# Krual-T/OutfitX

Hardware: AMD Instinct MI355X
Metric: outfits/sec CP forward (8-item sets, 224^2, bf16) (higher is better)
Workload: dtype f16

## Files before the change

outfitx_amd/csrc/fused_qkv_attn.hip:

```cpp
#include "attn_wave.h"
#include "gemm_common.h"

namespace {

struct FusedK {
    const char* X;
    const char* Wqkv;
    char* out;
    const float* bias;
    const float* row_stat;
    const float* col_sum;
    int n_img, S, Wm, heads, ldx, ldo, G, nwg;
    float scale;
    const char* W8 = nullptr; const char* scale8 = nullptr;
};

constexpr int FQ_TM = 256, FQ_TN = 192, FQ_STAGE = (FQ_TM + FQ_TN) * BK * 2;
constexpr int FQ_QK_ROW = 144;
constexpr int FQ_NT = 4;
static_assert(FQ_TN == 3 * ATTN_D && 16 * FQ_NT == ATTN_D, "the tail runs the attention core at NT = 4 on one head's 64 q, 64 k and 64 v columns");
constexpr int FQ_Q_OFF = 0, FQ_K_OFF = FQ_TM * FQ_QK_ROW, FQ_V_OFF = 2 * FQ_TM * FQ_QK_ROW;
constexpr int FQ_LDS = 2 * FQ_STAGE + 16 * ATTN_V_ROW;
constexpr int FQ2_BK = 32, FQ2_A = FQ_TM * FQ2_BK * 2, FQ2_W = FQ_TN * FQ2_BK * 2, FQ2_STAGE = FQ2_A + 2 * FQ2_W, FQ2_NST = 3;
constexpr int FQ2_LDS = FQ2_NST * FQ2_STAGE;
static_assert(FQ2_LDS >= FQ_LDS, "q | k | v image must fit the dual-weight stages");
constexpr int FQ8_A = FQ_TM * 32 * 2, FQ8_W = FQ_TN * 32 * 2, FQ8_STAGE = FQ8_A + FQ8_W, FQ8_NST = 4;
constexpr int FQ8_W8BASE = FQ8_NST * FQ8_STAGE, FQ8_W8 = FQ_TN * 128;
constexpr int FQ8_IMG = FQ8_STAGE, FQ8_CST = FQ8_IMG + FQ_LDS, FQ8_CST_WAVE = (2 * 64 + 2 * 96) * 4;
constexpr int FQ8_LDS = FQ8_CST + 8 * FQ8_CST_WAVE;
static_assert(FQ8_CST >= FQ8_W8BASE + FQ8_W8 && FQ8_IMG + 2 * FQ_STAGE >= FQ8_W8BASE + FQ8_W8, "the V pad rows and the constants lie behind everything LDS-DMA fills");
static_assert(FQ8_LDS <= 160 * 1024, "one block per CU");

template <typename T>
__device__ __forceinline__ void fq_attention(OFX_LDS char* lds, const FusedK& p, int wave, int lane, int m0, int head);

template <typename T, bool W2 = false>
__global__ __launch_bounds__(512, 2) void fused_qkv_attn_kernel(FusedK p) {
    typedef typename OpT<T>::v8 v8;
    typedef typename OpT<T>::v4 v4;
    extern __shared__ __attribute__((aligned(16))) char smem[];
    OFX_LDS char* lds = (OFX_LDS char*)smem;
    const int tid = threadIdx.x, lane = tid & 63;
    const int wave = __builtin_amdgcn_readfirstlane(tid >> 6);
    const int wr = wave >> 2, wc = wave & 3;

    const int bid = xcd_remap(blockIdx.x, p.nwg);
    const int hh = p.heads % 2 == 0 ? p.heads / 2 : p.heads, halves = p.heads / hh, per_unit = 6 * hh;
    const int unit = bid / per_unit, in_unit = bid % per_unit;
    const int grp = (unit / halves) * 6 + in_unit / hh, head = (unit % halves) * hh + in_unit % hh;
    if (grp * p.G >= p.n_img) return;
    const int M = p.n_img * p.S;
    const int m0 = grp * p.G * p.S;
    const int n_live_img = min(p.G, p.n_img - grp * p.G);

    f32x4 acc[8][3];
#pragma unroll
    for (int i = 0; i < 8; ++i)
#pragma unroll
        for (int j = 0; j < 3; ++j) acc[i][j] = f32x4{0.f, 0.f, 0.f, 0.f};
    const int fr = lane & 15, fq = lane >> 4;

    if constexpr (W2) {
    const PpLane32 L(lane);
    const int prow = L.prow, pchk = L.pchk;
    const char* a_base = p.X + (size_t)m0 * p.ldx * 2;
    const char* w_base = p.Wqkv + (size_t)head * 64 * (2 * p.Wm) * 2;
    unsigned a_off[2], w_off[3];
#pragma unroll
    for (int i = 0; i < 2; ++i) {
        const int row = (wave * 2 + i) * 16 + prow;
        const int rr = m0 + row < M ? row : M - 1 - m0;
        a_off[i] = ((unsigned)rr * p.ldx + pchk * 8) * 2;
    }
    int w_dst[3];
#pragma unroll
    for (int i = 0; i < 3; ++i) {
        const int q = wave * 3 + i;
        const int row = (q % 12) * 16 + prow;
        const unsigned grow = (unsigned)(row >> 6) * p.Wm + (row & 63);
        w_off[i] = (grow * (2 * p.Wm) + (q >= 12 ? p.Wm : 0) + pchk * 8) * 2;
        w_dst[i] = FQ2_A + (q >= 12 ? FQ2_W : 0) + (q % 12) * 1024;
    }
    const int a_dst = wave * 2 * 1024;
    const int nk = p.Wm / FQ2_BK;
    auto issue_all = [&](int step) {
        const int sc = step < nk ? step : nk - 1;
        OFX_LDS char* base = lds + (step % FQ2_NST) * FQ2_STAGE;
        const char* ak = a_base + (size_t)sc * FQ2_BK * 2;
        const char* wk = w_base + (size_t)sc * FQ2_BK * 2;
#pragma unroll
        for (int i = 0; i < 2; ++i) glds16(ak + a_off[i], base + a_dst + i * 1024);
#pragma unroll
        for (int i = 0; i < 3; ++i) glds16(wk + w_off[i], base + w_dst[i]);
    };
    const int a_frag = (wr * 128 + fr) * 64 + L.fchk;
    const int w_frag = FQ2_A + (wc * 48 + fr) * 64 + L.fchk;
    v8 af[8], wh[3], wl[3];
    auto read = [&](int t) { pp_w2_read<3>(lds + (t % FQ2_NST) * FQ2_STAGE, a_frag, w_frag, FQ2_W, af, wh, wl); };
    auto mfma = [&] { pp_w2_mfma<T, 3>(acc, af, wh, wl); };
    issue_all(0); issue_all(1);
    asm volatile("s_waitcnt vmcnt(5)" ::: "memory");
    __builtin_amdgcn_s_barrier();
    if (wr == 0) {
        for (int t = 0; t < nk; ++t) pp_slot<0, 5>([&] { issue_all(t + 2); }, [&] { read(t); }, mfma);
        pp_group_end<0>();
    } else {
        pp_group_begin<1>();
        for (int t = 0; t < nk; ++t) pp_slot<1, 5>([&] { issue_all(t + 2); }, [&] { read(t); }, mfma);
    }
    asm volatile("s_waitcnt vmcnt(0)" ::: "memory");
    __builtin_amdgcn_s_barrier();
    if (tid < 16 * ATTN_V_ROW / 16) *(OFX_LDS f32x4*)(lds + 2 * FQ_STAGE + tid * 16) = f32x4{0.f, 0.f, 0.f, 0.f};
    } else {
    if (tid < 16 * ATTN_V_ROW / 16) *(OFX_LDS f32x4*)(lds + 2 * FQ_STAGE + tid * 16) = f32x4{0.f, 0.f, 0.f, 0.f};

    const int lrow = lane >> 3, lchk = lane & 7;
    const char* a_base = p.X + (size_t)m0 * p.ldx * 2;
    const char* w_base = p.Wqkv + (size_t)head * 64 * p.Wm * 2;
    unsigned a_off[4], w_off[3];
#pragma unroll
    for (int i = 0; i < 4; ++i) {
        const int row = (wave * 4 + i) * 8 + lrow;
        const int rr = m0 + row < M ? row : M - 1 - m0;
        a_off[i] = ((unsigned)rr * p.ldx + (lchk ^ ((row >> 1) & 7)) * 8) * 2;
    }
#pragma unroll
    for (int i = 0; i < 3; ++i) {
        const int row = (wave * 3 + i) * 8 + lrow;
        const unsigned grow = (unsigned)(row >> 6) * p.Wm + (row & 63);
        w_off[i] = (grow * p.Wm + (lchk ^ ((row >> 1) & 7)) * 8) * 2;
    }
    const int a_dst = wave * 4 * 1024, w_dst = FQ_TM * BK * 2 + wave * 3 * 1024;
    auto issue_all = [&](int kt, int stage) {
        OFX_LDS char* base = lds + stage * FQ_STAGE;
        const char* ak = a_base + (size_t)kt * BK * 2;
        const char* wk = w_base + (size_t)kt * BK * 2;
#pragma unroll
        for (int i = 0; i < 4; ++i) glds16(ak + a_off[i], base + a_dst + i * 1024);
#pragma unroll
        for (int i = 0; i < 3; ++i) glds16(wk + w_off[i], base + w_dst + i * 1024);
    };

    const int fsw = fr >> 1;
    const int a_frag = (wr * 128 + fr) * 128;
    const int w_frag = FQ_TM * BK * 2 + (wc * 48 + fr) * 128;
    v8 af[2][8], wf[2][3];

#define FQ_READ_FRAGS(STG)                                                                                    \
    {                                                                                                         \
        OFX_LDS char* base_ = lds + (STG) * FQ_STAGE;                                                         \
        _Pragma("unroll") for (int ks = 0; ks < 2; ++ks) {                                                    \
            const int chk = ((ks * 4 + fq) ^ fsw) * 16;                                                       \
            _Pragma("unroll") for (int j = 0; j < 3; ++j) wf[ks][j] = *(OFX_LDS v8*)(base_ + w_frag + j * 16 * 128 + chk); \
            _Pragma("unroll") for (int i = 0; i < 8; ++i) af[ks][i] = *(OFX_LDS v8*)(base_ + a_frag + i * 16 * 128 + chk); \
        }                                                                                                     \
    }

    const int nk = p.Wm / BK;
    issue_all(0, 0);
    issue_all(nk > 1 ? 1 : 0, 1);
    asm volatile("s_waitcnt vmcnt(7)" ::: "memory");
    __builtin_amdgcn_s_barrier();
    if (wr == 0) {
        for (int t = 0; t < nk; ++t) {
            if (t >= 1 && t + 1 < nk) issue_all(t + 1, (t + 1) & 1);
            FQ_READ_FRAGS(t & 1)
            asm volatile("s_waitcnt lgkmcnt(0)" ::: "memory");
            __builtin_amdgcn_s_barrier();
            __builtin_amdgcn_s_setprio(1);
#pragma unroll
            for (int m = 0; m < 48; ++m) {
                const int ks = m / 24, i = (m % 24) / 3, j = m % 3;
                acc[i][j] = OpT<T>::mfma16(wf[ks][j], af[ks][i], acc[i][j]);
            }
            __builtin_amdgcn_s_setprio(0);
            asm volatile("s_waitcnt vmcnt(0)" ::: "memory");
            __builtin_amdgcn_s_barrier();
        }
        __builtin_amdgcn_s_barrier();
    } else {
        __builtin_amdgcn_s_barrier();
        for (int t = 0; t < nk; ++t) {
            FQ_READ_FRAGS(t & 1)
            asm volatile("s_waitcnt vmcnt(0)" ::: "memory");
            asm volatile("s_waitcnt lgkmcnt(0)" ::: "memory");
            __builtin_amdgcn_s_barrier();
            OFX_LDS char* nbase = lds + (t & 1) * FQ_STAGE;
            const int kn = t + 2 < nk ? t + 2 : nk - 1;
            const char* ak = a_base + (size_t)kn * BK * 2;
            const char* wk = w_base + (size_t)kn * BK * 2;
            __builtin_amdgcn_s_setprio(1);
#pragma unroll
            for (int m = 0; m < 48; ++m) {
                if (m % 6 == 0 && m / 6 < 7) {
                    const int q = m / 6;
                    if (q < 4) glds16(ak + a_off[q], nbase + a_dst + q * 1024);
                    else glds16(wk + w_off[q - 4], nbase + w_dst + (q - 4) * 1024);
                }
                const int ks = m / 24, i = (m % 24) / 3, j = m % 3;
                acc[i][j] = OpT<T>::mfma16(wf[ks][j], af[ks][i], acc[i][j]);
            }
            __builtin_amdgcn_s_setprio(0);
            __builtin_amdgcn_s_barrier();
        }
    }
#undef FQ_READ_FRAGS
    asm volatile("s_waitcnt vmcnt(0)" ::: "memory");
    __builtin_amdgcn_s_barrier();
    }

    {
        float mu[8], rs[8];
#pragma unroll
        for (int i = 0; i < 8; ++i) {
            mu[i] = 0.f; rs[i] = 1.f;
            if (p.row_stat) {
                const int gm = min(m0 + wr * 128 + i * 16 + fr, M - 1);
                const f32x2 ms = *(const f32x2*)(p.row_stat + 2 * (size_t)gm);
                mu[i] = ms[0]; rs[i] = ms[1];
            }
        }
#pragma unroll
        for (int j = 0; j < 3; ++j) {
            const int c = wc * 48 + j * 16 + fq * 4, which = c >> 6, d = c & 63;
            const int gn = which * p.Wm + head * 64 + d;
            const f32x4 b4 = *(const f32x4*)(p.bias + gn);
            f32x4 cs4 = {0.f, 0.f, 0.f, 0.f};
            if (p.row_stat) cs4 = *(const f32x4*)(p.col_sum + gn);
            OFX_LDS char* reg = lds + (which == 0 ? FQ_Q_OFF : which == 1 ? FQ_K_OFF : FQ_V_OFF);
            const int stride = which == 2 ? ATTN_V_ROW : FQ_QK_ROW;
#pragma unroll
            for (int i = 0; i < 8; ++i) {
                const int row = wr * 128 + i * 16 + fr;
                const f32x4 v = (acc[i][j] - cs4 * mu[i]) * rs[i] + b4;
                v4 o;
#pragma unroll
                for (int e = 0; e < 4; ++e) o[e] = (T)v[e];
                *(OFX_LDS v4*)(reg + row * stride + d * 2) = o;
            }
        }
    }
    asm volatile("s_waitcnt lgkmcnt(0)" ::: "memory");
    __builtin_amdgcn_s_barrier();

    if (wave >= n_live_img) return;
    fq_attention<T>(lds, p, wave, lane, m0, head);
}

template <typename T>
__device__ __forceinline__ void fq_attention(OFX_LDS char* lds, const FusedK& p, int wave, int lane, int m0, int head) {
    typedef typename OpT<T>::v8 v8;
    constexpr int NT = FQ_NT;
    const int S = p.S, r0 = wave * S;
    const int r16 = lane & 15, q4 = lane >> 4;
    OFX_LDS char* ql = lds + FQ_Q_OFF + r0 * FQ_QK_ROW;
    OFX_LDS char* kl = lds + FQ_K_OFF + r0 * FQ_QK_ROW;
    OFX_LDS char* vl = lds + FQ_V_OFF + r0 * ATTN_V_ROW;
    v8 kf[NT][2], qf[NT][2];
#pragma unroll
    for (int t = 0; t < NT; ++t) {
        int row = 16 * t + r16;
        row = row < S ? row : S - 1;
#pragma unroll
        for (int ks = 0; ks < 2; ++ks) {
            kf[t][ks] = *(OFX_LDS v8*)(kl + row * FQ_QK_ROW + (q4 * 8 + ks * 32) * 2);
            qf[t][ks] = *(OFX_LDS v8*)(ql + row * FQ_QK_ROW + (q4 * 8 + ks * 32) * 2);
        }
    }
    float neg[NT][4];
#pragma unroll
    for (int t = 0; t < NT; ++t)
#pragma unroll
        for (int r = 0; r < 4; ++r) neg[t][r] = (16 * t + 4 * q4 + r >= S) ? -INFINITY : 0.f;
    f32x4 st[NT][NT];
    attn_scores<T, NT>(st, kf, qf, neg, NT);
    v8 pf[NT][attn_ksteps(NT)];
    attn_softmax_p<T, NT, false>(pf, st, p.scale, NT);
    attn_pv_store<T, NT>(vl, pf, NT, true, (T*)p.out, m0 + r0, p.ldo, head * 64, S, 0);
}

typedef int fq_i32x8 __attribute__((ext_vector_type(8)));
typedef int fq_i32x4 __attribute__((ext_vector_type(4)));
typedef short fq_i16x2 __attribute__((ext_vector_type(2)));
typedef _Float16 fq_f16x2 __attribute__((ext_vector_type(2)));

__global__ __launch_bounds__(512, 2) void fused_qkv_attn_w2f8_kernel(FusedK p) {
    typedef f16_t T;
    typedef OpT<T>::v8 v8;
    typedef OpT<T>::v4 v4;
    constexpr int BK2 = 32, PART = FQ8_A, STAGE = FQ8_STAGE;
    extern __shared__ __attribute__((aligned(16))) char smem[];
    OFX_LDS char* lds = (OFX_LDS char*)smem;
    OFX_LDS char* img = lds + FQ8_IMG;
    const int tid = threadIdx.x, lane = tid & 63;
    const int wave = __builtin_amdgcn_readfirstlane(tid >> 6);
    const int wr = wave >> 1, wc = wave & 1;
    int grp = wave >> 2;
    asm volatile("" : "+s"(grp));
    const int Kh = p.Wm, nk = Kh / BK2, nsup = nk >> 2;
    const int M = p.n_img * p.S;
    const float a_scale = 1.0f;
    const int a_e8 = 127;

    const int hh = p.heads % 2 == 0 ? p.heads / 2 : p.heads, halves = p.heads / hh, per_unit = 6 * hh;
    auto decode = [&](int v, int& g, int& h) {
        const int bid = xcd_remap(v, p.nwg), unit = bid / per_unit, in_unit = bid % per_unit;
        g = (unit / halves) * 6 + in_unit / hh;
        h = (unit % halves) * hh + in_unit % hh;
    };
    auto next_live = [&](int v) {
        for (; v < p.nwg; v += (int)gridDim.x) {
            int g, h;
            decode(v, g, h);
            if (g * p.G < p.n_img) break;
        }
        return v;
    };
    int vb = next_live(blockIdx.x);
    if (vb >= p.nwg) return;

    int ln = lane;
    asm volatile("" : "+v"(ln));
    OFX_LDS float* cst = (OFX_LDS float*)(lds + FQ8_CST + wave * FQ8_CST_WAVE);

    auto load_consts = [&](int m0_, int head_, f32x2& ms, f32x4& c4, unsigned long long (&sw)[3]) {
        ms = f32x2{0.f, 1.f};
        c4 = f32x4{0.f, 0.f, 0.f, 0.f};
        if (p.row_stat) ms = *(const f32x2*)(p.row_stat + 2 * (size_t)min(m0_ + wr * 64 + ln, M - 1));
        const float* cb = ln >= 32 ? (p.row_stat ? p.col_sum : nullptr) : p.bias;
        const int c = wc * 96 + (ln & 31) * 4;
        if (cb && (ln & 31) < 24) c4 = *(const f32x4*)(cb + (c >> 6) * Kh + head_ * 64 + (c & 63));
#pragma unroll
        for (int w = 0; w < 3; ++w) sw[w] = *(const unsigned long long*)(p.scale8 + ((size_t)(w * (Kh >> 7) + (head_ >> 1)) * 16 + (ln & 15)) * 8);
    };
    auto stash_consts = [&](int head_, f32x2 ms, f32x4 c4, const unsigned long long (&sw)[3], int& sa, int& sb) {
        *(OFX_LDS f32x2*)(cst + 2 * ln) = ms;
        if ((ln & 31) < 24) *(OFX_LDS f32x4*)(cst + 128 + (ln >> 5) * 96 + (ln & 31) * 4) = c4;
        const int sh = (head_ & 1) * 32;
        const unsigned q_ = (unsigned)(sw[0] >> sh), k_ = (unsigned)(sw[1] >> sh), v_ = (unsigned)(sw[2] >> sh);
        sa = (int)(wc == 0 ? q_ : (k_ >> 16) | (v_ << 16));
        sb = (int)(wc == 0 ? k_ : v_ >> 16);
    };

    const size_t a_row = (size_t)p.ldx * 2;
    const unsigned w_head = 64u * (2 * Kh) * 2;
    const __amdgpu_buffer_rsrc_t r_w = make_rsrc(p.Wqkv), r_w8 = make_rsrc(p.W8);
    int grp_t, head, sc_a, sc_b;
    decode(vb, grp_t, head);
    {
        f32x2 ms; f32x4 c4; unsigned long long sw[3];
        load_consts(grp_t * p.G * p.S, head, ms, c4, sw);
        stash_consts(head, ms, c4, sw, sc_a, sc_b);
    }
    if (tid < 16 * ATTN_V_ROW / 16) *(OFX_LDS f32x4*)(img + 2 * FQ_STAGE + tid * 16) = f32x4{0.f, 0.f, 0.f, 0.f};
    bool first = true;

    for (;;) {
        const int vn = next_live(vb + (int)gridDim.x);
        const bool has_next = vn < p.nwg;
        int grp_n = grp_t, head_n = head;
        if (has_next) decode(vn, grp_n, head_n);
        const int m0 = grp_t * p.G * p.S, m1 = grp_n * p.G * p.S;
        const int n_live_img = min(p.G, p.n_img - grp_t * p.G);
        int l2 = ln;
        asm volatile("" : "+v"(l2));
        const PpLane32 L(l2);
        const int fr = L.fr, fq = L.fq;
        const int wp0 = grp == 0 ? wave * 2 : 4 + wave;
        unsigned a_off[2], w_off[2], w8_off[3];
#pragma unroll
        for (int i = 0; i < 2; ++i) {
            a_off[i] = ((unsigned)((wave * 2 + i) * 16 + L.prow) * p.ldx + L.pchk * 8) * 2;
            const int row = ((wp0 + i) * 16 + L.prow) % FQ_TN;
            w_off[i] = (((unsigned)(row >> 6) * Kh + (row & 63)) * (2 * Kh) + L.pchk * 8) * 2;
        }
#pragma unroll
        for (int q = 0; q < 3; ++q) {
            const int P = wave * 3 + q;
            w8_off[q] = (unsigned)((P >> 3) * Kh + (P & 7) * 8 + (l2 >> 3)) * Kh + ((((l2 & 7) ^ (((l2 >> 4) & 3) << 1)) ^ (P & 1)) << 4);
        }
        const int a_dst = wave * 2 * 1024, w_dst = PART + wp0 * 1024, w8_dst = FQ8_W8BASE + wave * 3 * 1024;
        const int a_frag = (wr * 64 + fr) * 64 + L.fchk;
        const int w_frag = PART + (wc * 96 + fr) * 64 + L.fchk;
        const int x8 = (((fr >> 1) & 3) << 1) | (fr >> 3);
        const int w8_frag0 = (wc * 96 + fr) * 128 + (((2 * fq) ^ x8) << 4), w8_frag1 = (wc * 96 + fr) * 128 + (((2 * fq + 1) ^ x8) << 4);
        const __amdgpu_buffer_rsrc_t r_a = make_rsrc(p.X + (size_t)m0 * a_row, (size_t)(M - m0) * a_row), r_a1 = make_rsrc(p.X + (size_t)m1 * a_row, (size_t)(M - m1) * a_row);
        auto issue_step = [&](int x, bool two_w) {
            OFX_LDS char* stg = lds + (x & 3) * STAGE;
            const bool nx = x == nk;
            const __amdgpu_buffer_rsrc_t ra = nx ? r_a1 : r_a;
            const unsigned koff = (unsigned)(nx ? 0 : (x > nk ? nk - 1 : x)) * BK2 * 2;
            const unsigned sw = (unsigned)(nx ? head_n : head) * w_head + koff;
            bload16(ra, a_off[0], koff, stg + a_dst); bload16(ra, a_off[1], koff, stg + a_dst + 1024);
            bload16(r_w, w_off[0], sw, stg + w_dst);
            if (two_w) bload16(r_w, w_off[1], sw, stg + w_dst + 1024);
        };
#define FQ8_ISSUE_W8(SUP, Q) bload16(r_w8, w8_off[Q], (unsigned)head * 64u * (unsigned)Kh + (unsigned)(SUP) * 128u, lds + w8_dst + (Q) * 1024);

        f32x4 acc[4][6];
#pragma unroll
        for (int i = 0; i < 4; ++i)
#pragma unroll
            for (int j = 0; j < 6; ++j) acc[i][j] = f32x4{0.f, 0.f, 0.f, 0.f};
        v8 af[4], wh[6];
        fq_i32x8 a8[4];
#pragma unroll
        for (int i = 0; i < 4; ++i) a8[i] = fq_i32x8{0, 0, 0, 0, 0, 0, 0, 0};
        auto read = [&](int step) {
            OFX_LDS char* stg = lds + (step & 3) * STAGE;
#pragma unroll
            for (int j = 0; j < 6; ++j) wh[j] = *(OFX_LDS v8*)(stg + w_frag + j * 16 * 64);
#pragma unroll
            for (int i = 0; i < 4; ++i) af[i] = *(OFX_LDS v8*)(stg + a_frag + i * 16 * 64);
        };
#define FQ8_CVT1(I, S)                                                                                        \
    {                                                                                                         \
        fq_i16x2 lo_ = __builtin_bit_cast(fq_i16x2, a8[I][2 * (S)]), hi_ = __builtin_bit_cast(fq_i16x2, a8[I][2 * (S) + 1]); \
        lo_ = __builtin_amdgcn_cvt_scalef32_pk_bf8_f16(lo_, fq_f16x2{af[I][0], af[I][1]}, a_scale, false);    \
        lo_ = __builtin_amdgcn_cvt_scalef32_pk_bf8_f16(lo_, fq_f16x2{af[I][2], af[I][3]}, a_scale, true);     \
        hi_ = __builtin_amdgcn_cvt_scalef32_pk_bf8_f16(hi_, fq_f16x2{af[I][4], af[I][5]}, a_scale, false);    \
        hi_ = __builtin_amdgcn_cvt_scalef32_pk_bf8_f16(hi_, fq_f16x2{af[I][6], af[I][7]}, a_scale, true);     \
        a8[I][2 * (S)] = __builtin_bit_cast(int, lo_); a8[I][2 * (S) + 1] = __builtin_bit_cast(int, hi_);      \
    }
#define FQ8_MFMA16(S)                                                                                         \
    {                                                                                                         \
        __builtin_amdgcn_s_setprio(1);                                                                        \
        _Pragma("unroll") for (int j = 0; j < 6; ++j) {                                                       \
            _Pragma("unroll") for (int i = 0; i < 4; ++i) acc[i][j] = OpT<T>::mfma16(wh[j], af[i], acc[i][j]); \
            if (j >= 2) FQ8_CVT1(j - 2, S)                                                                    \
        }                                                                                                     \
        __builtin_amdgcn_s_setprio(0);                                                                        \
    }
#define FQ8_LD(J)                                                                                             \
    {                                                                                                         \
        const fq_i32x4 c0_ = *(OFX_LDS fq_i32x4*)(b8_ + w8_frag0 + (J) * 16 * 128), c1_ = *(OFX_LDS fq_i32x4*)(b8_ + w8_frag1 + (J) * 16 * 128); \
        w8_[(J) % 3] = fq_i32x8{c0_[0], c0_[1], c0_[2], c0_[3], c1_[0], c1_[1], c1_[2], c1_[3]};              \
    }
#define FQ8_MF(J, SEL, SC)                                                                                    \
    if ((J) + 2 < 6) { FQ8_LD((J) + 2) __builtin_amdgcn_sched_barrier(0); }                                   \
    _Pragma("unroll") for (int i = 0; i < 4; ++i)                                                             \
        acc[i][J] = __builtin_amdgcn_mfma_scale_f32_16x16x128_f8f6f4(w8_[(J) % 3], a8[i], acc[i][J], 0, 1, SEL, SC, 0, a_e8);
#define FQ8_MFMA8()                                                                                           \
    {                                                                                                         \
        __builtin_amdgcn_sched_barrier(0);                                                                    \
        OFX_LDS char* b8_ = lds + FQ8_W8BASE;                                                                 \
        fq_i32x8 w8_[3];                                                                                      \
        FQ8_LD(0) FQ8_LD(1)                                                                                   \
        __builtin_amdgcn_s_setprio(1);                                                                        \
        FQ8_MF(0, 0, sc_a) FQ8_MF(1, 1, sc_a) FQ8_MF(2, 2, sc_a) FQ8_MF(3, 3, sc_a)                           \
        FQ8_MF(4, 0, sc_b) FQ8_MF(5, 1, sc_b)                                                                 \
        __builtin_amdgcn_s_setprio(0);                                                                        \
    }

        if (first) {
            issue_step(0, grp == 0); issue_step(1, grp == 0);
            if (grp == 0) asm volatile("s_waitcnt vmcnt(4)" ::: "memory");
            else { issue_step(2, false); asm volatile("s_waitcnt vmcnt(6)" ::: "memory"); }
        } else {
            issue_step(1, grp == 0);
            if (grp != 0) issue_step(2, false);
        }
        asm volatile("" : "+v"(sc_a), "+v"(sc_b));
        asm volatile("s_setreg_imm32_b32 hwreg(HW_REG_MODE, 23, 1), 1");
        __builtin_amdgcn_s_barrier();
        auto run = [&](auto G) {
            constexpr int g = G.value;
            constexpr bool w2 = g == 0;
            pp_group_begin<g>();
            int u = 0;
            do {
                const int t = 4 * u;
                pp_slot<g, g ? 3 : 8>([&] { if (g == 0) issue_step(t + 2, w2); issue_step(t + 3, w2); }, [&] { read(t); }, [&] { FQ8_MFMA16(0) });
                pp_slot<g, 3>([&] { FQ8_ISSUE_W8(u, 0) FQ8_ISSUE_W8(u, 1) FQ8_ISSUE_W8(u, 2) }, [&] { read(t + 1); }, [&] { FQ8_MFMA16(1) });
                pp_slot<g, g ? 3 : 4>([&] { issue_step(t + 4, w2); }, [&] { read(t + 2); }, [&] { FQ8_MFMA16(2) });
                pp_slot<g, g ? 6 : 4>([&] { issue_step(t + 5, w2); if (g == 1) issue_step(t + 6, w2); }, [&] { read(t + 3); }, [&] { FQ8_MFMA16(3) }, [&] { FQ8_MFMA8() });
            } while (++u < nsup);
            pp_group_end<g>();
        };
        if (grp == 0) run(std::integral_constant<int, 0>());
        else run(std::integral_constant<int, 1>());
#undef FQ8_MFMA16
#undef FQ8_MFMA8
#undef FQ8_MF
#undef FQ8_LD
#undef FQ8_CVT1
#undef FQ8_ISSUE_W8
        asm volatile("s_setreg_imm32_b32 hwreg(HW_REG_MODE, 23, 1), 0");
        asm volatile("s_waitcnt vmcnt(0)" ::: "memory");
        __builtin_amdgcn_s_barrier();

        f32x2 ms_n; f32x4 c4_n; unsigned long long sw_n[3];
        load_consts(m1, head_n, ms_n, c4_n, sw_n);

        {
            const KArgs none{};
            auto emit = [&](auto FOLD) {
                constexpr bool fold = FOLD.value;
#pragma unroll
                for (int j = 0; j < 6; ++j) {
                    const int c = wc * 96 + j * 16 + fq * 4, which = c >> 6, d = c & 63;
                    const f32x4 b4 = *(OFX_LDS const f32x4*)(cst + 128 + j * 16 + fq * 4);
                    f32x4 cs4 = {0.f, 0.f, 0.f, 0.f};
                    if (fold) cs4 = *(OFX_LDS const f32x4*)(cst + 224 + j * 16 + fq * 4);
                    OFX_LDS char* reg = img + (which == 0 ? FQ_Q_OFF : which == 1 ? FQ_K_OFF : FQ_V_OFF);
                    const int stride = which == 2 ? ATTN_V_ROW : FQ_QK_ROW;
#pragma unroll
                    for (int i = 0; i < 4; ++i) {
                        const int row = wr * 64 + i * 16 + fr;
                        float mu = 0.f, rs = 1.f;
                        if (fold) { const f32x2 ms = *(OFX_LDS const f32x2*)(cst + 2 * (i * 16 + fr)); mu = ms[0]; rs = ms[1]; }
                        const f32x4 v = epi_value(none, acc[i][j], OFX_ACT_NONE, fold, mu, rs, cs4, b4, false);
                        v4 o;
#pragma unroll
                        for (int e = 0; e < 4; ++e) o[e] = (T)v[e];
                        *(OFX_LDS v4*)(reg + row * stride + d * 2) = o;
                    }
                }
            };
            if (p.row_stat) emit(std::true_type());
            else emit(std::false_type());
        }
        stash_consts(head_n, ms_n, c4_n, sw_n, sc_a, sc_b);
        asm volatile("s_waitcnt lgkmcnt(0)" ::: "memory");
        __builtin_amdgcn_s_barrier();

        if (wave < n_live_img) fq_attention<T>(img, p, wave, ln, m0, head);
        if (!has_next) break;
        __builtin_amdgcn_s_barrier();
        vb = vn; grp_t = grp_n; head = head_n;
        first = false;
    }
}

}

int ofx_launch_fused_qkv_attn(const void* X, const void* Wqkv, const float* bias, const float* row_stat, const float* col_sum, void* out,
                              int n_img, int S, int Wm, int heads, int ldx, int ldo, float scale, int op_dtype, hipStream_t s, FusedQkvForm form,
                              const void* W8, const void* scale8) {
    const bool w2 = form != FUSED_QKV_PLAIN, f8 = form == FUSED_QKV_W2F8;
    OFX_REQUIRE(X && Wqkv && bias && out && n_img > 0, OFX_EINVAL, "fused_qkv_attn: NULL argument");
    OFX_REQUIRE(!f8 || (W8 && scale8), OFX_EINVAL, "fused_qkv_attn: the fp8 form needs W8 and scale8");
    OFX_REQUIRE(!f8 || op_dtype == OFX_F16, OFX_EINVAL, "fused_qkv_attn: the fp8 form takes f16 operands");
    OFX_REQUIRE(S >= 33 && S <= 64 && Wm == heads * 64 && Wm % BK == 0 && Wm / BK >= 2, OFX_ESHAPE, "fused_qkv_attn: S=%d must be in [33,64], width %d = heads * 64", S, Wm);
    OFX_REQUIRE(!f8 || Wm % 128 == 0, OFX_ESHAPE, "fused_qkv_attn: the fp8 form needs a width that is a multiple of 128, not %d", Wm);
    OFX_REQUIRE(!f8 || ((size_t)FQ_TM * ldx * 2 < 0x7fffffff && (size_t)3 * Wm * Wm * 4 < 0x7fffffff), OFX_ESHAPE, "fused_qkv_attn: the fp8 form takes weights below 2 GiB");
    OFX_REQUIRE((FQ_TM / S - 1) * S + 64 - FQ_TM <= 16, OFX_ESHAPE, "fused_qkv_attn: S=%d would read %d key rows past the tile's 16 pad rows (supported: 33, 34, 37..41, 43..64)", S,
                (FQ_TM / S - 1) * S + 64 - FQ_TM);
    OFX_REQUIRE(ldx >= Wm && ldx % 8 == 0 && ldo >= Wm && ldo % 8 == 0, OFX_ESHAPE, "fused_qkv_attn: bad strides");
    OFX_REQUIRE(!row_stat || col_sum, OFX_EINVAL, "fused_qkv_attn: row_stat needs col_sum");
    FusedK k;
    k.X = (const char*)X; k.Wqkv = (const char*)Wqkv; k.out = (char*)out; k.bias = bias; k.row_stat = row_stat; k.col_sum = col_sum;
    k.n_img = n_img; k.S = S; k.Wm = Wm; k.heads = heads; k.ldx = ldx; k.ldo = ldo; k.G = FQ_TM / S; k.scale = scale;
    k.W8 = (const char*)W8; k.scale8 = (const char*)scale8;
    const int groups = (n_img + k.G - 1) / k.G;
    k.nwg = ((groups + 5) / 6) * 6 * heads;
    static DeviceOnce attr;
    TRY(attr.run([]() -> int {
        OFX_HIP(hipFuncSetAttribute((const void*)fused_qkv_attn_kernel<bf16_t, false>, hipFuncAttributeMaxDynamicSharedMemorySize, FQ_LDS));
        OFX_HIP(hipFuncSetAttribute((const void*)fused_qkv_attn_kernel<f16_t, false>, hipFuncAttributeMaxDynamicSharedMemorySize, FQ_LDS));
        OFX_HIP(hipFuncSetAttribute((const void*)fused_qkv_attn_kernel<bf16_t, true>, hipFuncAttributeMaxDynamicSharedMemorySize, FQ2_LDS));
        OFX_HIP(hipFuncSetAttribute((const void*)fused_qkv_attn_kernel<f16_t, true>, hipFuncAttributeMaxDynamicSharedMemorySize, FQ2_LDS));
        OFX_HIP(hipFuncSetAttribute((const void*)fused_qkv_attn_w2f8_kernel, hipFuncAttributeMaxDynamicSharedMemorySize, FQ8_LDS));
        return OFX_OK;
    }));
    const double wbytes = f8 ? 3.0 : (w2 ? 4.0 : 2.0), products = f8 ? 1.5 : (w2 ? 2.0 : 1.0);
    if (g_ofx_prof_on) ofx_prof_set_tag(n_img * S, 3 * Wm, Wm, 7, w2 ? 2 : 1, 2.0 * n_img * S * Wm + wbytes * 3.0 * Wm * Wm + 2.0 * n_img * S * Wm);
    ProfScope prof(PROF_GEMM, s, products * 2.0 * n_img * S * 3.0 * Wm * Wm + 4.0 * n_img * S * S * Wm, true);
    if (f8) {
        OFX_PLAUNCH(true, fused_qkv_attn_w2f8_kernel, dim3(ofx_gemm_w2_grid(k.nwg)), dim3(512), FQ8_LDS, s, k);
    } else if (w2) {
        if (op_dtype == OFX_F16) OFX_PLAUNCH(true, (fused_qkv_attn_kernel<f16_t, true>), dim3(k.nwg), dim3(512), FQ2_LDS, s, k);
        else OFX_PLAUNCH(true, (fused_qkv_attn_kernel<bf16_t, true>), dim3(k.nwg), dim3(512), FQ2_LDS, s, k);
    } else {
        if (op_dtype == OFX_F16) OFX_PLAUNCH(true, (fused_qkv_attn_kernel<f16_t, false>), dim3(k.nwg), dim3(512), FQ_LDS, s, k);
        else OFX_PLAUNCH(true, (fused_qkv_attn_kernel<bf16_t, false>), dim3(k.nwg), dim3(512), FQ_LDS, s, k);
    }
    OFX_LAUNCH_CHECK();
    return OFX_OK;
}
```

Measured before the change: 8260.

## Split attention tail across all waves by query tiles instead of per image

The attention tail previously ran one whole image per wave, leaving waves beyond the live image count idle. It now divides the (image, 16-row query tile) units evenly across all 8 waves, each running up to two runs of 1–3 query tiles with templated attention helpers. This spreads the tail's work over idle waves at the cost of reloading K/V fragments per run and extra code variants that raise register pressure.

```diff
diff --git a/outfitx_amd/csrc/fq_units.h b/outfitx_amd/csrc/fq_units.h
--- /dev/null
+++ b/outfitx_amd/csrc/fq_units.h
@@ -0,0 +1,20 @@
+#pragma once
+
+constexpr int FQ_UNITS_MAX = 3;
+
+struct FqWaveUnits {
+    int img, q0, n0, n1;
+};
+
+constexpr int fq_live_qtiles(int S) { return (S + 15) >> 4; }
+
+constexpr FqWaveUnits fq_wave_units(int wave, int n_live_img, int lq) {
+    const int units = n_live_img * lq, s = wave & 3;
+    const int a = (s * units) >> 2, b = ((s + 1) * units) >> 2;
+    const int mid = a + ((b - a + 1) >> 1);
+    const int lo = wave < 4 ? a : mid, hi = wave < 4 ? mid : b;
+    const int img = lq == 4 ? lo >> 2 : lo / 3;
+    const int q0 = lo - img * lq;
+    const int n0 = hi - lo < lq - q0 ? hi - lo : lq - q0;
+    return FqWaveUnits{img, q0, n0, hi - lo - n0};
+}
diff --git a/outfitx_amd/csrc/fused_qkv_attn.hip b/outfitx_amd/csrc/fused_qkv_attn.hip
--- a/outfitx_amd/csrc/fused_qkv_attn.hip
+++ b/outfitx_amd/csrc/fused_qkv_attn.hip
@@ -1,4 +1,5 @@
 #include "attn_wave.h"
+#include "fq_units.h"
 #include "gemm_common.h"
 
 namespace {
@@ -32,7 +33,7 @@
 static_assert(FQ8_LDS <= 160 * 1024, "one block per CU");
 
 template <typename T>
-__device__ __forceinline__ void fq_attention(OFX_LDS char* lds, const FusedK& p, int wave, int lane, int m0, int head);
+__device__ __forceinline__ void fq_attention(OFX_LDS char* lds, const FusedK& p, int wave, int lane, int m0, int head, int n_live_img);
 
 template <typename T, bool W2 = false>
 __global__ __launch_bounds__(512, 2) void fused_qkv_attn_kernel(FusedK p) {
@@ -243,40 +244,59 @@
     asm volatile("s_waitcnt lgkmcnt(0)" ::: "memory");
     __builtin_amdgcn_s_barrier();
 
-    if (wave >= n_live_img) return;
-    fq_attention<T>(lds, p, wave, lane, m0, head);
+    fq_attention<T>(lds, p, wave, lane, m0, head, n_live_img);
 }
 
-template <typename T>
-__device__ __forceinline__ void fq_attention(OFX_LDS char* lds, const FusedK& p, int wave, int lane, int m0, int head) {
+template <typename T, int NU>
+__device__ __forceinline__ void fq_attention_run(OFX_LDS char* lds, const FusedK& p, int lane, int m0, int head, int r0, int q0) {
     typedef typename OpT<T>::v8 v8;
     constexpr int NT = FQ_NT;
-    const int S = p.S, r0 = wave * S;
+    const int S = p.S;
     const int r16 = lane & 15, q4 = lane >> 4;
     OFX_LDS char* ql = lds + FQ_Q_OFF + r0 * FQ_QK_ROW;
     OFX_LDS char* kl = lds + FQ_K_OFF + r0 * FQ_QK_ROW;
     OFX_LDS char* vl = lds + FQ_V_OFF + r0 * ATTN_V_ROW;
-    v8 kf[NT][2], qf[NT][2];
+    v8 kf[NT][2], qf[NU][2];
 #pragma unroll
     for (int t = 0; t < NT; ++t) {
         int row = 16 * t + r16;
         row = row < S ? row : S - 1;
 #pragma unroll
-        for (int ks = 0; ks < 2; ++ks) {
-            kf[t][ks] = *(OFX_LDS v8*)(kl + row * FQ_QK_ROW + (q4 * 8 + ks * 32) * 2);
-            qf[t][ks] = *(OFX_LDS v8*)(ql + row * FQ_QK_ROW + (q4 * 8 + ks * 32) * 2);
-        }
+        for (int ks = 0; ks < 2; ++ks) kf[t][ks] = *(OFX_LDS v8*)(kl + row * FQ_QK_ROW + (q4 * 8 + ks * 32) * 2);
+    }
+#pragma unroll
+    for (int u = 0; u < NU; ++u) {
+        int row = 16 * (q0 + u) + r16;
+        row = row < S ? row : S - 1;
+#pragma unroll
+        for (int ks = 0; ks < 2; ++ks) qf[u][ks] = *(OFX_LDS v8*)(ql + row * FQ_QK_ROW + (q4 * 8 + ks * 32) * 2);
     }
     float neg[NT][4];
 #pragma unroll
     for (int t = 0; t < NT; ++t)
 #pragma unroll
         for (int r = 0; r < 4; ++r) neg[t][r] = (16 * t + 4 * q4 + r >= S) ? -INFINITY : 0.f;
-    f32x4 st[NT][NT];
-    attn_scores<T, NT>(st, kf, qf, neg, NT);
-    v8 pf[NT][attn_ksteps(NT)];
-    attn_softmax_p<T, NT, false>(pf, st, p.scale, NT);
-    attn_pv_store<T, NT>(vl, pf, NT, true, (T*)p.out, m0 + r0, p.ldo, head * 64, S, 0);
+    f32x4 st[NT][NU];
+    attn_scores<T, NT, NU>(st, kf, qf, neg, NU);
+    v8 pf[NU][attn_ksteps(NT)];
+    attn_softmax_p<T, NT, false, NU>(pf, st, p.scale, NU);
+    attn_pv_store<T, NT, NU>(vl, pf, NU, true, (T*)p.out, m0 + r0 + 16 * q0, p.ldo, head * 64, S - 16 * q0, 0);
+}
+
+template <typename T>
+__device__ __forceinline__ void fq_attention(OFX_LDS char* lds, const FusedK& p, int wave, int lane, int m0, int head, int n_live_img) {
+    const FqWaveUnits w = fq_wave_units(wave, n_live_img, fq_live_qtiles(p.S));
+#pragma unroll 1
+    for (int run = 0; run < 2; ++run) {
+        const int n = run ? w.n1 : w.n0, r0 = (w.img + run) * p.S, q0 = run ? 0 : w.q0;
+        static_assert(FQ_UNITS_MAX == 3, "one case per run length");
+        switch (n) {
+            case 1: fq_attention_run<T, 1>(lds, p, lane, m0, head, r0, q0); break;
+            case 2: fq_attention_run<T, 2>(lds, p, lane, m0, head, r0, q0); break;
+            case 3: fq_attention_run<T, 3>(lds, p, lane, m0, head, r0, q0); break;
+            default: return;
+        }
+    }
 }
 
 typedef int fq_i32x8 __attribute__((ext_vector_type(8)));
@@ -524,7 +544,7 @@
         asm volatile("s_waitcnt lgkmcnt(0)" ::: "memory");
         __builtin_amdgcn_s_barrier();
 
-        if (wave < n_live_img) fq_attention<T>(img, p, wave, ln, m0, head);
+        fq_attention<T>(img, p, wave, ln, m0, head, n_live_img);
         if (!has_next) break;
         __builtin_amdgcn_s_barrier();
         vb = vn; grp_t = grp_n; head = head_n;
```

Result: no change. 8279, median of 6 (+0.2%).
